# Schatten2021/rust-raytracing

Measured on AMD Instinct MI355X. Metric: Mrays/s (primary rays, whole node), 10k-sphere 1080p 64spp, higher is better.
Workload: dtype f64; 1 GPU; C2: 10k random spheres (scene seed 1), 1920x1080, 64 spp; width=1920, height=1080, rays_per_pixel=64, n_objects=10000, partition=single GPU

## Files before the change

rust-raytracing_amd/csrc/rtx_api.hip:

```cpp
#include "../../include/rtx_hip.h"
#include "rtx_launch.h"

#include <cmath>
#include <cstdio>
#include <cstdlib>
#include <cstring>
#include <string>
#include <thread>
#include <vector>

using namespace rtx;

namespace {

thread_local std::string g_last_error;

int32_t fail(RtxStatus st, const std::string &msg)
{
    g_last_error = msg;
    return (int32_t)st;
}

#define RTX_HIP_CHECK(expr)                                                                              \
    do {                                                                                                 \
// ... 334 lines not shown
        }
        n_in_tree = bvh.tri_order.size();
    } else {
        for (size_t k = 0; k < all_tree.size(); ++k) (all_free[k] == 2 ? demoted : always_recs).push_back(all_tree[k]);
    }
    p.sv.n_tri_tree = (uint32_t)n_in_tree;
    for (const TriRec &r : demoted) { tri32.push_back(r.A); tri32.push_back(r.B); tri_fidx.push_back(r.tri); }
    for (const TriRec &r : always_recs) { tri32.push_back(r.A); tri32.push_back(r.B); tri_fidx.push_back(r.tri); }
    if (!tri32.empty()) {
        tri32.push_back(make_float4(0.f, 0.f, 0.f, 0.f));
        tri32.push_back(make_float4(0.f, 0.f, 0.f, 0.f));
    }
    p.sv.n_tri_filter = (uint32_t)tri_fidx.size();
    p.sv.tri_extent = tri_extent;
    p.sv.n_objects = (uint32_t)n;
    p.sv.n_spheres = (uint32_t)spheres.size();
    p.sv.n_planes = (uint32_t)planes.size();
    p.sv.n_tris = (uint32_t)tris.size();
    for (int c = 0; c < 3; ++c) p.sv.sphere_center[c] = centre[c];
    p.sv.sphere_cmax = cmax;

    p.sv.n_bvh_nodes = (uint32_t)bvh4.nodes.size();
    p.sv.bvh_depth = (uint32_t)bvh4.depth;
    p.sv.bvh_root = bvh4.root;
    p.sv.bvh_origin_limit = (float)bvh.origin_limit;
    p.sv.bvh_inv_max = (float)std::fmin(1.0e30, 1.0e37 / std::fmax(bvh.origin_limit, 1.0));
    p.sv.bvh_flags = (bvh.has_spheres ? 1u : 0u) | (bvh.has_tris ? 2u : 0u) |
                     (bvh.has_tris && !bvh.has_spheres && tree_recs[1].empty() && tree_recs[0].empty() ? 4u : 0u);
    if ((p.sv.bvh_flags & 4u) && build_qnodes(bvh4, p.qnodes)) p.sv.bvh_flags |= 8u;
    else p.qnodes.clear();
#ifndef RTX_LAB
    if ((p.sv.bvh_flags & 12u) == 4u) p.sv.bvh_flags &= ~4u;
#endif
    if ((p.sv.bvh_flags & 3u) == 1u && build_q3nodes(bvh4, bvh.abs_pad, p.q3nodes)) p.sv.bvh_flags |= 16u;
    else p.q3nodes.clear();
    if (debug_prints())
        std::fprintf(stderr, "[rtx_hip] upload: %zu spheres, %zu triangles (%zu in the tree: %zu xy / %zu xz / %zu yz footprints, %zu tested per segment), bvh: %zu binary nodes, %zu wide nodes, depth %d\n",
                     spheres.size(), tris.size(), n_in_tree, tree_recs[2].size(), tree_recs[1].size(), tree_recs[0].size(),
                     demoted.size() + always_recs.size(), bvh.nodes.size(), bvh4.nodes.size(), bvh4.depth);
    std::vector<float4> &leaf32 = p.leaf32;
    leaf32.assign(bvh.prims.size(), make_float4(0.f, 0.f, 0.f, 0.f));
    for (size_t k = 0; k < bvh.prims.size(); ++k) {
        const uint32_t p = bvh.prims[k];
        leaf32[k] = make_float4(fx[p], fy[p], fz[p], fw[p]);
    }
    p.leaf_cr.assign(bvh.prims.size(), make_float4(0.f, 0.f, 0.f, 0.f));
    for (size_t k = 0; k < bvh.prims.size(); ++k) {
        const uint32_t q = bvh.prims[k];
        p.leaf_cr[k] = make_float4(fx[q], fy[q], fz[q], round_up_f32(std::fabs(scene->objects[sphere_id[q]].geom[3])));
    }

    return RTX_OK;
}

int32_t upload_packed(RtxSceneHandle_ *h, const PackedScene &p)
{
    const SceneView sv_before = h->sv;
    std::vector<void *> old_allocs;
    old_allocs.swap(h->scene_allocs);
    {
        SceneView sv = p.sv;
        sv.rays_per_pixel = h->sv.rays_per_pixel; sv.max_bounces = h->sv.max_bounces;
        sv.focal_length = h->sv.focal_length; sv.focal_offset = h->sv.focal_offset; sv.non_focal_offset = h->sv.non_focal_offset;
        sv.seed = h->sv.seed; sv.tuning = h->sv.tuning;
        h->sv = sv;
    }
    h->sv.cam_pos = mk(h->cam.position[0], h->cam.position[1], h->cam.position[2]);
// ... 919 lines not shown
            const Bvh4Node &w = p.bvh4.nodes[k];
            const BvhQNode &q = p.qnodes[k];
            const float lk[4] = { w.b[0].x, w.b[0].y, w.b[0].z, w.b[0].w }, ct[4] = { w.b[1].x, w.b[1].y, w.b[1].z, w.b[1].w };
            for (int c = 0; c < 4; ++c) {
                const uint32_t count = bits(ct[c]), type = q.link[c] >> kQNodeShift;
                if ((count == 0xFFFFFFFFu) != (type == kQNodeEmpty)) return fail(RTX_ERR_INVALID_ARGUMENT, "bvh check: quantised node: empty slot differs");
                if (type == kQNodeEmpty) continue;
                if ((q.link[c] & kQNodeIndexMask) != (bits(lk[c]) & ~kBvhFlatNode) || (type == 0u) != (count == 0u) ||
                    (type != 0u && type != (count & 0xFFFFu)))
                    return fail(RTX_ERR_INVALID_ARGUMENT, "bvh check: quantised node: link / count differs");
                const double lx = (double)q.ox + (double)(q.qx[c] & 0xFFFFu) * q.sx, hx = (double)q.ox + (double)(q.qx[c] >> 16) * q.sx;
                const double ly = (double)q.oy + (double)(q.qy[c] & 0xFFFFu) * q.sy, hy = (double)q.oy + (double)(q.qy[c] >> 16) * q.sy;
                if (!(lx <= (double)w.a[c].x && ly <= (double)w.a[c].y && hx >= (double)w.a[c].z && hy >= (double)w.a[c].w))
                    return fail(RTX_ERR_INVALID_ARGUMENT, "bvh check: quantised rectangle does not contain the child's");
            }
        }
        stats[15] = p.qnodes.size();
    }
    if (p.sv.bvh_flags & 16u) {
        if (p.q3nodes.size() != n_nodes) return fail(RTX_ERR_INVALID_ARGUMENT, "bvh check: 64-byte sphere node count differs");
        for (size_t k = 0; k < n_nodes; ++k) {
            const Bvh4Node &w = p.bvh4.nodes[k];
            const BvhQ3Node &q = p.q3nodes[k];
            const uint32_t *lows[3] = { &q.lox, &q.loy, &q.loz }, *highs[3] = { &q.hix, &q.hiy, &q.hiz };
            const float org[3] = { q.ox, q.oy, q.oz }, stp[3] = { q.sx, q.sy, q.sz };
            for (int c = 0; c < 4; ++c) {
                const uint32_t count = bits(w.b[c].w), type = q.link[c] >> kQNodeShift;
                if ((count == 0xFFFFFFFFu) != (type == kQNodeEmpty)) return fail(RTX_ERR_INVALID_ARGUMENT, "bvh check: 64-byte sphere node: empty slot differs");
                if (type == kQNodeEmpty) continue;
                if ((q.link[c] & kQNodeIndexMask) != bits(w.a[c].w) || (type == 0u) != (count == 0u) || (type != 0u && type != count))
                    return fail(RTX_ERR_INVALID_ARGUMENT, "bvh check: 64-byte sphere node: link / count differs");
                const float l[3] = { w.a[c].x, w.a[c].y, w.a[c].z }, hh[3] = { w.b[c].x, w.b[c].y, w.b[c].z };
                for (int a = 0; a < 3; ++a) {
                    const float dl = std::fmaf((float)((*lows[a] >> (8 * c)) & 255u), stp[a], org[a]);
                    const float dh = std::fmaf((float)((*highs[a] >> (8 * c)) & 255u), stp[a], org[a]);
                    if (!((double)dl <= (double)l[a] - p.bvh.abs_pad * 0.999 && (double)dh >= (double)hh[a] + p.bvh.abs_pad * 0.999))
                        return fail(RTX_ERR_INVALID_ARGUMENT, "bvh check: decoded 64-byte box does not contain the child's (+ pad)");
                }
            }
        }
        stats[15] = p.q3nodes.size();
    }
    if (depth != p.bvh4.depth) return fail(RTX_ERR_INVALID_ARGUMENT, "bvh check: recorded depth differs");
    for (size_t k = 0; k < n_nodes; ++k) if (!node_seen[k]) return fail(RTX_ERR_INVALID_ARGUMENT, "bvh check: unreachable node");
    if ((p.sv.bvh_flags & 1u) && stats[8] != p.spheres.size()) return fail(RTX_ERR_INVALID_ARGUMENT, "bvh check: a sphere is in no leaf");
    if ((p.sv.bvh_flags & 2u) && stats[9] != p.sv.n_tri_tree) return fail(RTX_ERR_INVALID_ARGUMENT, "bvh check: a triangle is in no leaf");
    return RTX_OK;
}

int32_t rtx_debug_paths(RtxSceneHandle h, uint32_t width, uint32_t height, uint32_t row, uint32_t max_steps, RtxPathStep *steps,
                        uint32_t *counts)
{
#ifdef RTX_LAB
    static_assert(sizeof(RtxPathStep) == sizeof(PathStep) && sizeof(PathStep) == 64, "RtxPathStep layout");
    if (!h || !steps || !counts) return fail(RTX_ERR_INVALID_ARGUMENT, "rtx_debug_paths: null argument");
    if (width == 0 || row >= height || max_steps == 0) return fail(RTX_ERR_INVALID_ARGUMENT, "rtx_debug_paths: bad row / size");
    const uint64_t paths = (uint64_t)width * h->cfg.rays_per_pixel;
    if (paths == 0) return RTX_OK;
    if (paths * max_steps > (1ull << 24)) return fail(RTX_ERR_INVALID_ARGUMENT, "rtx_debug_paths: more than 2^24 steps asked for");
    RTX_HIP_CHECK(hipSetDevice(h->device));
    struct Bufs {
        RtxSceneHandle_ *h; double *rgb = nullptr; uint32_t kernel;
        ~Bufs() {
            (void)hipDeviceSynchronize();
            if (h->transcript) (void)hipFree(h->transcript);
            if (h->transcript_counts) (void)hipFree(h->transcript_counts);
            if (rgb) (void)hipFree(rgb);
            h->transcript = nullptr; h->transcript_counts = nullptr; h->transcript_steps = 0; h->cfg.kernel = kernel;
        }
// ... 44 lines not shown
```

rust-raytracing_amd/csrc/rtx_bvh.h:

```cpp
#pragma once

#include <hip/hip_runtime.h>
#include <stdint.h>

#include <algorithm>
#include <cmath>
#include <cstring>
#include <numeric>
#include <vector>

namespace rtx {

struct BvhNode {
    float lo[3];
    uint32_t link;
    float hi[3];
    uint32_t count;
};
static_assert(sizeof(BvhNode) == 32, "BvhNode must be 32 bytes");

constexpr uint32_t kBvhTriLeaf = 0x10000u;
constexpr int kBvhLeafSize = 1;
constexpr int kBvhTriLeafMax = 8;

// ... 376 lines not shown
        }
        BvhQNode q;
        double o[2], sc[2];
        for (int a = 0; a < 2; ++a) {
            o[a] = std::isfinite(lo[a]) ? lo[a] : 0.0;
            const double ext = std::isfinite(lo[a]) ? hi[a] - lo[a] : 0.0;
            sc[a] = ext > 0.0 ? std::exp2(std::ceil(std::log2(ext / 65535.0))) : 1.0;
            while (ext / sc[a] > 65535.0) sc[a] *= 2.0;
            if (!(sc[a] >= 1.1754944e-38 && sc[a] <= 1.0e30)) return false;
        }
        q.ox = (float)o[0]; q.oy = (float)o[1]; q.sx = (float)sc[0]; q.sy = (float)sc[1];
        for (int c = 0; c < 4; ++c) {
            if (ct[c] == 0xFFFFFFFFu) { q.qx[c] = 0x0000FFFFu; q.qy[c] = 0x0000FFFFu; q.link[c] = kQNodeEmpty << kQNodeShift; continue; }
            const double l0 = std::floor(((double)w.a[c].x - o[0]) / sc[0]), h0 = std::ceil(((double)w.a[c].z - o[0]) / sc[0]);
            const double l1 = std::floor(((double)w.a[c].y - o[1]) / sc[1]), h1 = std::ceil(((double)w.a[c].w - o[1]) / sc[1]);
            if (l0 < 0 || l1 < 0 || h0 > 65535 || h1 > 65535) return false;
            q.qx[c] = (uint32_t)l0 | ((uint32_t)h0 << 16);
            q.qy[c] = (uint32_t)l1 | ((uint32_t)h1 << 16);
            uint32_t type;
            if (ct[c] == 0u) type = 0u;
            else if ((ct[c] & kBvhTriLeaf) && (ct[c] & 0xFFFFu) >= 1u && (ct[c] & 0xFFFFu) <= kQNodeLeafMax) type = ct[c] & 0xFFFFu;
            else return false;
            const uint32_t idx = lk[c] & ~kBvhFlatNode;
            if (idx > kQNodeIndexMask) return false;
            if (type == 0u && !(lk[c] & kBvhFlatNode)) return false;
            q.link[c] = (type << kQNodeShift) | idx;
        }
        out.push_back(q);
    }
    return true;
}


struct BvhQ3Node {
    float ox, oy, oz, sx;
    float sy, sz;
    uint32_t lox, loy;
    uint32_t loz, hix, hiy, hiz;
    uint32_t link[4];
};
static_assert(sizeof(BvhQ3Node) == 64, "BvhQ3Node must be 64 bytes");

inline bool build_q3nodes(const Bvh4Build &b4, double abs_pad, std::vector<BvhQ3Node> &out)
{
    out.clear();
    out.reserve(b4.nodes.size());
    auto bits = [](float f) { uint32_t u; std::memcpy(&u, &f, 4); return u; };
    for (const Bvh4Node &w : b4.nodes) {
        double lo[3] = { INFINITY, INFINITY, INFINITY }, hi[3] = { -INFINITY, -INFINITY, -INFINITY };
        uint32_t cnt[4], lnk[4];
        for (int c = 0; c < 4; ++c) {
            cnt[c] = bits(w.b[c].w); lnk[c] = bits(w.a[c].w);
            if (cnt[c] == 0xFFFFFFFFu) continue;
            const float l[3] = { w.a[c].x, w.a[c].y, w.a[c].z }, h[3] = { w.b[c].x, w.b[c].y, w.b[c].z };
            for (int a = 0; a < 3; ++a) {
                if (!std::isfinite(l[a]) || !std::isfinite(h[a])) return false;
                lo[a] = std::min(lo[a], (double)l[a] - abs_pad); hi[a] = std::max(hi[a], (double)h[a] + abs_pad);
            }
        }
        BvhQ3Node q;
        std::memset(&q, 0, sizeof q);
        double o[3], sc[3];
        for (int a = 0; a < 3; ++a) {
            const double ext = std::isfinite(lo[a]) ? hi[a] - lo[a] : 0.0;
            sc[a] = ext > 0.0 ? std::exp2(std::ceil(std::log2(ext / 254.0))) : 1.0;
            if (!(sc[a] >= 1.1754944e-38 && sc[a] <= 1.0e30)) return false;
            o[a] = std::isfinite(lo[a]) ? std::floor(lo[a] / sc[a]) * sc[a] : 0.0;
            while (std::isfinite(lo[a]) && (hi[a] - o[a]) / sc[a] > 255.0) { sc[a] *= 2.0; o[a] = std::floor(lo[a] / sc[a]) * sc[a]; }
            if (!(std::fabs(o[a] / sc[a]) + 256.0 < 16777216.0)) return false;
            if ((double)(float)o[a] != o[a]) return false;
        }
        q.ox = (float)o[0]; q.oy = (float)o[1]; q.oz = (float)o[2]; q.sx = (float)sc[0]; q.sy = (float)sc[1]; q.sz = (float)sc[2];
        uint32_t *lows[3] = { &q.lox, &q.loy, &q.loz }, *highs[3] = { &q.hix, &q.hiy, &q.hiz };
        for (int c = 0; c < 4; ++c) {
            if (cnt[c] == 0xFFFFFFFFu) {
                for (int a = 0; a < 3; ++a) *lows[a] |= 255u << (8 * c);
                q.link[c] = kQNodeEmpty << kQNodeShift;
                continue;
            }
            const float l[3] = { w.a[c].x, w.a[c].y, w.a[c].z }, h[3] = { w.b[c].x, w.b[c].y, w.b[c].z };
            for (int a = 0; a < 3; ++a) {
                const double ql = std::floor(((double)l[a] - abs_pad - o[a]) / sc[a]), qh = std::ceil(((double)h[a] + abs_pad - o[a]) / sc[a]);
                if (ql < 0 || qh > 255 || ql > qh) return false;
                *lows[a] |= (uint32_t)ql << (8 * c);
                *highs[a] |= (uint32_t)qh << (8 * c);
            }
            uint32_t type;
            if (cnt[c] == 0u) type = 0u;
            else if ((cnt[c] & kBvhTriLeaf) == 0u && cnt[c] >= 1u && cnt[c] <= kQNodeLeafMax) type = cnt[c];
            else return false;
            if (lnk[c] > kQNodeIndexMask || (lnk[c] & kBvhFlatNode)) return false;
            q.link[c] = (type << kQNodeShift) | lnk[c];
        }
        out.push_back(q);
    }
    return true;
}

}
```

rust-raytracing_amd/csrc/rtx_bvh_spheres_lab.h:

```cpp
#pragma once

constexpr int kPoolSlots = 128;
constexpr int kPoolStack = kSphStack - 1;
constexpr uint32_t kPoolFresh = 1u << 10, kPoolNoWalk = 1u << 9, kPoolOverflow = 1u << 8;
#ifndef RTX_POOL_SERVE
#define RTX_POOL_SERVE 24
#endif
#ifndef RTX_POOL_WAIT
#define RTX_POOL_WAIT 8
#endif
constexpr uint32_t kPoolWait = RTX_POOL_WAIT;
constexpr uint32_t kPoolServe = RTX_POOL_SERVE;
constexpr int kPoolF64 = 13, kPoolU32 = 28;
struct SphPool {
    double *f;
    uint32_t *u;
    size_t stride;
};

size_t bvh_spheres_pool2_bytes(int n_cus)
{
    const size_t slots = (size_t)n_cus * kSphWavesPerSimd * (kBvhThreads / 64) * kPoolSlots;
    return slots * (kPoolF64 * sizeof(double) + kPoolU32 * sizeof(uint32_t)) + 512;
}
// ... 886 lines not shown
                rec->d = make_double4(__longlong_as_double((long long)r.key),
                                      __longlong_as_double((long long)(((unsigned long long)r.bounce << 32) | (unsigned long long)ridx)), 0.0, 0.0);
                if (nowalk) { sl[9 * kSlotN + my] = kSlotNoWalk; sl[8 * kSlotN + my] = __float_as_uint(__builtin_inff()); }
            } else if (have && !dead) {
                sl[9 * kSlotN + my] = kSlotFresh;
            }
            const bool to_ready = go && !nowalk, to_done = have && !dead && !to_ready;
            const unsigned long long rm = __ballot(to_ready), dm = __ballot(to_done);
            if (to_ready) ready_list[n_ready + bvh_mbcnt(rm)] = (uint8_t)my;
            if (to_done) done_list[n_done + bvh_mbcnt(dm)] = (uint8_t)my;
            n_ready += (uint32_t)__popcll(rm);
            n_done += (uint32_t)__popcll(dm);
#ifndef RTX_SLOT_NOFENCE
            __threadfence_block();
#endif
            { RTX_SLOT_T(t_s2) RTX_SLOT_ACC(2, t_s1, t_s2) }
            continue;
        }
        if (n_idle == 64u) break;
        for (;;) {
            const bool w = walking && node != kNone;
            const bool at_leaf = w && (node >> 29) != 0u;
            const unsigned long long lm = __ballot(at_leaf), am = __ballot(w);
            if (am == 0ull) break;
            if ((uint32_t)__popcll(lm) >= kSphLeafLanes || lm == am) {
                if (at_leaf)
                    sphere_leaf_step_at<STACK, SPILL, kSlotN>(la.sphere_f32, la.sphere_prims, sr, node, sp, &lds_stack[0][0], sl, tid, slot, spill,
                                                              spill_stride, glane, best_up, qcnt, overflow, nleaf);
            } else if (w && !at_leaf) {
#if defined(RTX_LAB) && defined(RTX_SLOT_COUNT_TOP)
                if (node < (uint32_t)(RTX_SLOT_COUNT_TOP)) exact += 1;
#endif
                sphere_node_step_q3<STACK, SPILL>(qnodes, q, node, sp, &lds_stack[0][0], tid, spill, spill_entries, spill_stride, glane, best_up,
                                                  overflow, nbox, kSlotTop > 0 ? (LdsF4Ptr)&lds_top[0] : (LdsF4Ptr) nullptr, top_n);
            }
            const uint32_t n_fin = (uint32_t)__popcll(__ballot(walking && node == kNone));
            if (n_fin >= kSlotWait) break;
        }
        { RTX_SLOT_T(t_s3) RTX_SLOT_ACC(1, t_s1, t_s3) }
    }
#ifdef RTX_SLOT_PROFILE
    exact = sp_prof;
#endif
    unsigned long long box_tests = nbox, filt = (unsigned long long)nbox + nleaf, segs64 = segs;
#pragma unroll
    for (int off = 32; off > 0; off >>= 1) {
        segs64 += __shfl_xor(segs64, off, 64);
        exact += __shfl_xor(exact, off, 64);
        filt += __shfl_xor(filt, off, 64);
        box_tests += __shfl_xor(box_tests, off, 64);
    }
    if (lane == 0) {
        const uint32_t shard = (blockIdx.x * (kBvhThreads >> 6) + (tid >> 6)) & (kCounterShards - 1);
        if (segs64) atomicAdd(&ctr[shard].segments, segs64);
        if (exact) atomicAdd(&ctr[shard].exact_tests, exact);
        if (filt) atomicAdd(&ctr[shard].filter_tests, filt);
        if (box_tests) atomicAdd(&ctr[2 + (shard % (kCounterShards - 2))].pad_, box_tests);
    }
}


static hipError_t launch_sph_lab_stage2(const SceneView *d_sv, const SceneView &sv, const RowsView *d_rv, const RowsView &rv, double *samples,
                                        Counters *counters, uint32_t *spill, uint32_t spill_entries, int n_cus, char *p, uint64_t capacity,
                                        unsigned long long *ctrs, SphQueue &sq, const LeafArrays &la, const float4 *nodes, uint32_t flags,
                                        void *pool_mem, hipStream_t stream)
{
    (void)rv;
// ... 53 lines not shown
```

rust-raytracing_amd/csrc/rtx_kernels.hip:

```cpp
#include "rtx_launch.h"
#include "rtx_traverse.h"

#include <cstdlib>

namespace rtx {

__device__ __forceinline__ uint32_t lane_id() { return __builtin_amdgcn_mbcnt_hi(~0u, __builtin_amdgcn_mbcnt_lo(~0u, 0u)); }

__device__ __forceinline__ uint32_t mbcnt(unsigned long long mask)
{
    return __builtin_amdgcn_mbcnt_hi((uint32_t)(mask >> 32), __builtin_amdgcn_mbcnt_lo((uint32_t)mask, 0u));
}

__device__ __forceinline__ unsigned long long wave_sum_u64(unsigned long long v)
{
#pragma unroll
    for (int off = 32; off > 0; off >>= 1) v += __shfl_xor(v, off, 64);
    return v;
}

__device__ __forceinline__ void flush_counters(Counters *ctr, unsigned long long segs, unsigned long long exact,
                                               unsigned long long filt)
{
    segs = wave_sum_u64(segs);
// ... 487 lines not shown
}

template <class T>
__global__ __launch_bounds__(256) void deinterleave_kernel(const T *__restrict__ parts, T *__restrict__ full,
                                                           uint32_t width, uint32_t height, uint32_t n, uint32_t cap_rows,
                                                           uint32_t block, uint32_t flip)
{
    const uint64_t i = (uint64_t)blockIdx.x * blockDim.x + threadIdx.x;
    const uint64_t row_vals = (uint64_t)width * 3;
    if (i >= row_vals * height) return;
    const uint32_t yo = (uint32_t)(i / row_vals);
    const uint64_t c = i - (uint64_t)yo * row_vals;
    const uint32_t y = flip ? height - 1u - yo : yo;
    const uint32_t b = y / block, p = b % n, k = (b / n) * block + (y - b * block);
    full[i] = parts[((uint64_t)p * cap_rows + k) * row_vals + c];
}

#ifdef RTX_LAB
__global__ void debug_math_kernel(int op, const double *a, const double *b, double *out, uint64_t n)
{
    uint64_t i = (uint64_t)blockIdx.x * blockDim.x + threadIdx.x;
    if (i >= n) return;
    double r;
    switch (op) {
        case 0: r = a[i] / b[i]; break;
        case 1: r = sqrt(a[i]); break;
        case 2: r = sin(a[i]); break;
        case 3: r = cos(a[i]); break;
        case 4: case 5: { double sn, cs; sincos(a[i], &sn, &cs); r = (op == 4) ? sn : cs; } break;
        case 6:
            r = (double)rtx_writelane(__builtin_amdgcn_readfirstlane((int)b[0]), __builtin_amdgcn_readfirstlane((int)b[1]), (int)a[i]);
            break;
        case 9: case 10: { double sn, cs; sincos_2pi(a[i], &sn, &cs); r = (op == 9) ? sn : cs; } break;
        default: {
            double lo, hi;
            rtx_minmax_f64_bits(a[i], b[i], lo, hi);
            r = (op == 7) ? lo : hi;
        } break;
    }
    out[i] = r;
}
#endif

hipError_t launch_trace_exact(const SceneView *d_sv, const RowsView *d_rv, const RowsView &rv, double *samples,
                              Counters *counters, hipStream_t stream)
{
    const uint64_t per_launch = 1ull << 30;
    for (uint64_t off = 0; off < rv.n_rays; off += per_launch) {
        uint64_t n = rv.n_rays - off < per_launch ? rv.n_rays - off : per_launch;
        uint32_t blocks = (uint32_t)((n + 255) / 256);
        hipLaunchKernelGGL(trace_exact_kernel, dim3(blocks), dim3(256), 0, stream, d_sv, d_rv, samples, counters, off);
        hipError_t e = hipGetLastError();
        if (e != hipSuccess) return e;
    }
    return hipSuccess;
}

namespace {

struct MixVariant {
    int s, threads, chunk, q, blocks_per_cu;
    size_t lds;
    const void *fn;
};

template <int S, int T, int CH, int Q, int WPE, int BPC>
// ... 126 lines not shown
```

rust-raytracing_amd/csrc/rtx_traverse.h:

```cpp
#pragma once

#include "rtx_device.h"

namespace rtx {

constexpr int kBvhThreads = 256;
constexpr uint32_t kNone = 0xFFFFFFFFu;
constexpr float kBvhRange64 = 134217728.0f;

struct Ray32 { float ix, iy, iz, nx, ny, nz; };
struct Ray64 { double ix, iy, iz, nx, ny, nz; };
struct Ray32S { float ix, iy, iz, nx, ny, nz, e; };
__device__ __forceinline__ float ray_slack(const Ray32 &) { return 0.0f; }
__device__ __forceinline__ float ray_slack(const Ray32S &r) { return r.e; }

__device__ __forceinline__ void ray32_axis(double o, double dn, double inv_max, float &inv, float &noi)
{
    double i = 1.0 / dn;
    if (!(fabs(i) <= inv_max)) i = copysign(inv_max, dn);
    inv = (float)i;
    noi = (float)(-o * (double)inv);
}

__device__ __forceinline__ void make_ray32(const V3 &pos, const V3 &dirn, double inv_max, Ray32 &r)
// ... 72 lines not shown
}

__device__ __forceinline__ float round_up32(double best)
{
    float b = (float)best;
    if ((double)b < best) b = __uint_as_float(__float_as_uint(b) + (b >= 0.0f ? 1u : 0xFFFFFFFFu));
    return b;
}

typedef float PkF4 __attribute__((ext_vector_type(4)));
typedef const __attribute__((address_space(3))) PkF4 *LdsF4Ptr;
struct PkConst4 {
    const __attribute__((address_space(4))) PkF4 *p;
    __device__ __forceinline__ PkConst4 operator+(size_t i) const { return PkConst4{p + i}; }
    __device__ __forceinline__ float4 operator[](size_t i) const { const PkF4 v = p[i]; return make_float4(v.x, v.y, v.z, v.w); }
};
__device__ __forceinline__ PkConst4 pk_const(const float4 *p) { return PkConst4{(const __attribute__((address_space(4))) PkF4 *)(uintptr_t)p}; }
__device__ __forceinline__ uint32_t pk_bits(float f) { return __builtin_amdgcn_readfirstlane(__float_as_uint(f)); }
struct PkConstU32 {
    const __attribute__((address_space(4))) uint32_t *p;
    __device__ __forceinline__ uint32_t operator[](size_t i) const { return p[i]; }
};
__device__ __forceinline__ PkConstU32 pk_const(const uint32_t *p) { return PkConstU32{(const __attribute__((address_space(4))) uint32_t *)(uintptr_t)p}; }

#if !defined(RTX_WRITELANE_VALIDATED) && defined(__clang_major__)
static_assert(__clang_major__ == 22, "rtx_writelane binds llvm.amdgcn.writelane.i32 by name: validated with AMD clang 22 (ROCm 7.2) only");
#endif
extern "C" __device__ int rtx_writelane(int value, int lane, int old) __asm("llvm.amdgcn.writelane.i32");

__device__ __forceinline__ void rtx_minmax_f64_bits(double a, double b, double &lo, double &hi)
{
    asm("v_min_f64 %0, %1, %2" : "=v"(lo) : "v"(a), "v"(b));
    asm("v_max_f64 %0, %1, %2" : "=v"(hi) : "v"(a), "v"(b));
}

constexpr int kBvhQueue = 8;
constexpr uint32_t kQueueTri = 0x80000000u;

struct LeafArrays {
    const float4 *sphere_f32;
    const uint32_t *sphere_prims;
    const SphereX *spheres;
    const uint32_t *sphere_ids;
    const float4 *tri_f32;
    const uint32_t *tri_fidx;
    const TriX *tris;
};

template <bool TRIS>
__device__ __forceinline__ void flush_candidates(const LeafArrays &la, const RayX &rx, const uint32_t *lds_q, uint32_t tid,
                                                 uint32_t &qcnt, Hit &h, float &best_up, unsigned long long &exact)
{
#pragma unroll 1
    for (uint32_t k = 0; k < qcnt; ++k) {
        const uint32_t idx = lds_q[(size_t)k * kBvhThreads + tid];
        double t;
        if (TRIS && (idx & kQueueTri)) {
            const uint32_t tk = la.tri_fidx[idx & ~kQueueTri];
            if (triangle_distance(la.tris[tk], rx, &t)) hit_consider(h, t, la.tris[tk].id, 2, tk);
        } else {
            if (sphere_distance(la.spheres[idx], rx, &t)) hit_consider(h, t, la.sphere_ids[idx], 0, idx);
        }
    }
    exact += qcnt;
    qcnt = 0;
    if (h.id != kNone) best_up = round_up32(h.t);
// ... 235 lines not shown
    node = key[0] < __builtin_inff() ? lnk[0] : kNone;
    if (node == kNone && sp != 0u) {
        sp -= 1;
        node = (!SPILL || sp < (uint32_t)STACK) ? lds_stack[(size_t)sp * kBvhThreads + tid]
                                                : spill[(size_t)(sp - (uint32_t)STACK) * spill_stride + glane];
    }
}

#ifndef RTX_Q3_SORT64
#define RTX_Q3_SORT64 1
#endif
template <int STACK, bool SPILL, class RAY>
__device__ __forceinline__ void sphere_step_q3(const float4 *__restrict__ qnodes, const float4 *__restrict__ leaf_f32,
                                               const uint32_t *__restrict__ leaf_prims, const RAY &q, const SphereRay &sr,
                                               uint32_t &node, uint32_t &sp, uint32_t *lds_stack, uint32_t *lds_q,
                                               uint32_t tid, uint32_t *__restrict__ spill, uint32_t spill_entries,
                                               size_t spill_stride, size_t glane, float &best_up, uint32_t &qcnt, bool &overflow,
                                               uint32_t &nbox, uint32_t &nleaf)
{
    const float4 *np = qnodes + 4 * (size_t)node;
    const float4 h0 = np[0], h1 = np[1], h2 = np[2], h3 = np[3];
    const float Sx = h0.w * q.ix, Sy = h1.x * q.iy, Sz = h1.y * q.iz;
    const float Ox = __builtin_fmaf(h0.x, q.ix, q.nx), Oy = __builtin_fmaf(h0.y, q.iy, q.ny), Oz = __builtin_fmaf(h0.z, q.iz, q.nz);
    const uint32_t lox = __float_as_uint(h1.z), loy = __float_as_uint(h1.w), loz = __float_as_uint(h2.x);
    const uint32_t hix = __float_as_uint(h2.y), hiy = __float_as_uint(h2.z), hiz = __float_as_uint(h2.w);
    const uint32_t lk[4] = { __float_as_uint(h3.x), __float_as_uint(h3.y), __float_as_uint(h3.z), __float_as_uint(h3.w) };
    const float e = ray_slack(q);
    float tc[4];
    uint32_t lnk[4], typ[4];
    const bool gx = q.ix < 0.0f, gy = q.iy < 0.0f, gz = q.iz < 0.0f;
    const uint32_t nxw = gx ? hix : lox, fxw = gx ? lox : hix;
    const uint32_t nyw = gy ? hiy : loy, fyw = gy ? loy : hiy;
    const uint32_t nzw = gz ? hiz : loz, fzw = gz ? loz : hiz;
#pragma unroll
    for (int c = 0; c < 4; ++c) {
        const float x0 = __builtin_fmaf((float)((nxw >> (8 * c)) & 255u), Sx, Ox), x1 = __builtin_fmaf((float)((fxw >> (8 * c)) & 255u), Sx, Ox);
        const float y0 = __builtin_fmaf((float)((nyw >> (8 * c)) & 255u), Sy, Oy), y1 = __builtin_fmaf((float)((fyw >> (8 * c)) & 255u), Sy, Oy);
        const float z0 = __builtin_fmaf((float)((nzw >> (8 * c)) & 255u), Sz, Oz), z1 = __builtin_fmaf((float)((fzw >> (8 * c)) & 255u), Sz, Oz);
        const float tn = fmaxf(fmaxf(x0, y0), fmaxf(z0, 0.0f));
        const float tf = fminf(fminf(x1, y1), z1);
        const float tn_lo = __builtin_fmaf(tn, 1.0f - 4.76837158e-7f, -e);
        const float tf_hi = __builtin_fmaf(tf, 1.0f + 4.76837158e-7f, e);
        typ[c] = lk[c] >> 29;
        lnk[c] = lk[c] & 0x1FFFFFFFu;
        tc[c] = (tn_lo <= tf_hi && tn_lo <= best_up && typ[c] != 7u) ? tn_lo : __builtin_inff();
    }
    nbox += 4;
    uint32_t leafmask = 0;
#pragma unroll
    for (int c = 0; c < 4; ++c)
        if (tc[c] < __builtin_inff() && typ[c] != 0u) leafmask |= 1u << c;
    while (leafmask != 0u) {
        const uint32_t c = (uint32_t)__builtin_ctz(leafmask);
        leafmask &= leafmask - 1u;
        const uint32_t first = c == 0 ? lnk[0] : (c == 1 ? lnk[1] : (c == 2 ? lnk[2] : lnk[3]));
        const uint32_t n = c == 0 ? typ[0] : (c == 1 ? typ[1] : (c == 2 ? typ[2] : typ[3]));
        for (uint32_t k = 0; k < n; ++k) {
            const float4 rec = leaf_f32[first + k];
            const float ox = rec.x - sr.px, oy = rec.y - sr.py, oz = rec.z - sr.pz;
            const float b = __builtin_fmaf(ox, sr.dx, __builtin_fmaf(oy, sr.dy, oz * sr.dz));
            const float lx = __builtin_fmaf(-b, sr.dx, ox), ly = __builtin_fmaf(-b, sr.dy, oy), lz = __builtin_fmaf(-b, sr.dz, oz);
            const float l2 = __builtin_fmaf(lx, lx, __builtin_fmaf(ly, ly, lz * lz));
            const float Dl = __builtin_fmaf(rec.w, rec.w, -l2);
            const float G = __builtin_fmaf(sr.Kg, rec.w, sr.c0);
            const float Dp = Dl + G;
            if (Dp >= 0.0f) {
                const float tlo = b - __builtin_amdgcn_sqrtf(Dp) * (1.0f + 4.76837158e-7f) - sr.K;
                const float Dm = Dl - G;
                const float thi = Dm > 0.0f ? b - __builtin_amdgcn_sqrtf(Dm) * (1.0f - 4.76837158e-7f) + sr.K : __builtin_inff();
                if (tlo <= best_up && !(thi < 0.0f)) {
                    if (tlo > sr.K) best_up = fminf(best_up, thi);
                    if (qcnt == (uint32_t)kSphQueue) {
                        uint32_t w = 0;
// ... 52 lines not shown
            if (sp < (uint32_t)STACK) { lds_stack[(size_t)sp * kBvhThreads + tid] = (v); sp += 1; } \
            else if (SPILL && sp - (uint32_t)STACK < spill_entries) {                                \
                spill[(size_t)(sp - (uint32_t)STACK) * spill_stride + glane] = (v); sp += 1;         \
            } else overflow = true;                                                                  \
        }
        if (key[3] < __builtin_inff()) RTX_PUSH(lnk[3])
        if (key[2] < __builtin_inff()) RTX_PUSH(lnk[2])
        if (key[1] < __builtin_inff()) RTX_PUSH(lnk[1])
#undef RTX_PUSH
    }
    node = key[0] < __builtin_inff() ? lnk[0] : kNone;
    if (node == kNone && sp != 0u) {
        sp -= 1;
        node = (!SPILL || sp < (uint32_t)STACK) ? lds_stack[(size_t)sp * kBvhThreads + tid]
                                                : spill[(size_t)(sp - (uint32_t)STACK) * spill_stride + glane];
    }
}

template <int STACK, bool SPILL, class RAY>
__device__ __forceinline__ void bvh_traverse_spheres(const float4 *__restrict__ nodes, const float4 *__restrict__ leaf_f32,
                                                     const uint32_t *__restrict__ leaf_prims, const RAY &q, const SphereRay &sr,
                                                     uint32_t root, uint32_t *lds_stack, uint32_t *lds_q,
                                                     uint32_t tid, uint32_t *__restrict__ spill, uint32_t spill_entries,
                                                     size_t spill_stride, size_t glane, float &best_up, uint32_t &qcnt, bool &overflow,
                                                     uint32_t &nbox, uint32_t &nleaf)
{
    uint32_t sp = 0;
    uint32_t node = root;
    while (node != kNone)
        sphere_step<STACK, SPILL>(nodes, leaf_f32, leaf_prims, q, sr, node, sp, lds_stack, lds_q, tid, spill, spill_entries,
                                  spill_stride, glane, best_up, qcnt, overflow, nbox, nleaf);
}

template <int STACK, bool SPILL, class RAY>
__device__ __forceinline__ void sphere_node_step_q3(const float4 *__restrict__ qnodes, const RAY &q, uint32_t &node, uint32_t &sp,
                                                    uint32_t *lds_stack, uint32_t tid, uint32_t *__restrict__ spill,
                                                    uint32_t spill_entries, size_t spill_stride, size_t glane, float best_up,
                                                    bool &overflow, uint32_t &nbox, LdsF4Ptr lds_top = nullptr, uint32_t top_n = 0u)
{
    float4 h0, h1, h2, h3;
    if (lds_top != nullptr && node < top_n) {
        LdsF4Ptr lp = lds_top + 4 * node;
        const PkF4 v0 = lp[0], v1 = lp[1], v2 = lp[2], v3 = lp[3];
        h0 = make_float4(v0.x, v0.y, v0.z, v0.w); h1 = make_float4(v1.x, v1.y, v1.z, v1.w);
        h2 = make_float4(v2.x, v2.y, v2.z, v2.w); h3 = make_float4(v3.x, v3.y, v3.z, v3.w);
    } else {
        const float4 *np = qnodes + 4 * (size_t)node;
        h0 = np[0]; h1 = np[1]; h2 = np[2]; h3 = np[3];
    }
    const float Sx = h0.w * q.ix, Sy = h1.x * q.iy, Sz = h1.y * q.iz;
    const float Ox = __builtin_fmaf(h0.x, q.ix, q.nx), Oy = __builtin_fmaf(h0.y, q.iy, q.ny), Oz = __builtin_fmaf(h0.z, q.iz, q.nz);
    const uint32_t lox = __float_as_uint(h1.z), loy = __float_as_uint(h1.w), loz = __float_as_uint(h2.x);
    const uint32_t hix = __float_as_uint(h2.y), hiy = __float_as_uint(h2.z), hiz = __float_as_uint(h2.w);
    const uint32_t lk[4] = { __float_as_uint(h3.x), __float_as_uint(h3.y), __float_as_uint(h3.z), __float_as_uint(h3.w) };
    const float e = ray_slack(q);
    const bool gx = q.ix < 0.0f, gy = q.iy < 0.0f, gz = q.iz < 0.0f;
    const uint32_t nxw = gx ? hix : lox, fxw = gx ? lox : hix;
    const uint32_t nyw = gy ? hiy : loy, fyw = gy ? loy : hiy;
    const uint32_t nzw = gz ? hiz : loz, fzw = gz ? loz : hiz;
    double kd[4];
#pragma unroll
    for (int c = 0; c < 4; ++c) {
        const float x0 = __builtin_fmaf((float)((nxw >> (8 * c)) & 255u), Sx, Ox), x1 = __builtin_fmaf((float)((fxw >> (8 * c)) & 255u), Sx, Ox);
        const float y0 = __builtin_fmaf((float)((nyw >> (8 * c)) & 255u), Sy, Oy), y1 = __builtin_fmaf((float)((fyw >> (8 * c)) & 255u), Sy, Oy);
        const float z0 = __builtin_fmaf((float)((nzw >> (8 * c)) & 255u), Sz, Oz), z1 = __builtin_fmaf((float)((fzw >> (8 * c)) & 255u), Sz, Oz);
        const float tn = fmaxf(fmaxf(x0, y0), fmaxf(z0, 0.0f));
        const float tf = fminf(fminf(x1, y1), z1);
        const float tn_lo = __builtin_fmaf(tn, 1.0f - 4.76837158e-7f, -e);
        const float tf_hi = __builtin_fmaf(tf, 1.0f + 4.76837158e-7f, e);
        const bool enter = (tn_lo <= fminf(tf_hi, best_up)) & (lk[c] < 0xE0000000u);
        const float key = enter ? tn_lo : __builtin_inff();
        kd[c] = __hiloint2double((int)__float_as_uint(key), (int)lk[c]);
    }
    nbox += 4;
#define RTX_CSWAP(i, j) { double lo_, hi_; rtx_minmax_f64_bits(kd[i], kd[j], lo_, hi_); kd[i] = lo_; kd[j] = hi_; }
    RTX_CSWAP(0, 1) RTX_CSWAP(2, 3) RTX_CSWAP(0, 2) RTX_CSWAP(1, 3) RTX_CSWAP(1, 2)
#undef RTX_CSWAP
    float key[4];
    uint32_t lnk[4];
#pragma unroll
    for (int c = 0; c < 4; ++c) { key[c] = __uint_as_float((uint32_t)__double2hiint(kd[c])); lnk[c] = (uint32_t)__double2loint(kd[c]); }
    const uint32_t npush = (key[1] < __builtin_inff() ? 1u : 0u) + (key[2] < __builtin_inff() ? 1u : 0u) +
                           (key[3] < __builtin_inff() ? 1u : 0u);
    if (sp + 3u <= (uint32_t)STACK) {
#pragma unroll
        for (uint32_t i = 1; i <= 3; ++i) {
            const uint32_t row = i <= npush ? sp + npush - i : (uint32_t)STACK;
            lds_stack[(size_t)row * kBvhThreads + tid] = lnk[i];
        }
        sp += npush;
    } else {
#define RTX_PUSH(v)                                                                                  \
        {                                                                                            \
            if (sp < (uint32_t)STACK) { lds_stack[(size_t)sp * kBvhThreads + tid] = (v); sp += 1; } \
            else if (SPILL && sp - (uint32_t)STACK < spill_entries) {                                \
                spill[(size_t)(sp - (uint32_t)STACK) * spill_stride + glane] = (v); sp += 1;         \
            } else overflow = true;                                                                  \
        }
        if (key[3] < __builtin_inff()) RTX_PUSH(lnk[3])
        if (key[2] < __builtin_inff()) RTX_PUSH(lnk[2])
        if (key[1] < __builtin_inff()) RTX_PUSH(lnk[1])
#undef RTX_PUSH
    }
    node = key[0] < __builtin_inff() ? lnk[0] : kNone;
    if (node == kNone && sp != 0u) {
// ... 51 lines not shown
    nleaf += n;
    node = kNone;
    if (sp != 0u) {
        sp -= 1;
        node = (!SPILL || sp < (uint32_t)STACK) ? lds_stack[(size_t)sp * kBvhThreads + tid]
                                                : spill[(size_t)(sp - (uint32_t)STACK) * spill_stride + glane];
    }
}

template <int STACK, bool SPILL>
__device__ __forceinline__ void sphere_leaf_step(const float4 *__restrict__ leaf_f32, const uint32_t *__restrict__ leaf_prims,
                                                 const SphereRay &sr, uint32_t &node, uint32_t &sp, uint32_t *lds_stack, uint32_t *lds_q,
                                                 uint32_t tid, uint32_t *__restrict__ spill, size_t spill_stride, size_t glane,
                                                 float &best_up, uint32_t &qcnt, bool &overflow, uint32_t &nleaf)
{
    sphere_leaf_step_at<STACK, SPILL, kBvhThreads>(leaf_f32, leaf_prims, sr, node, sp, lds_stack, lds_q, tid, tid, spill, spill_stride, glane,
                                                   best_up, qcnt, overflow, nleaf);
}

#if defined(RTX_LAB) && defined(RTX_SPH_PROFILE)
#define RTX_PROF_ARG , unsigned long long &rtx_prof
#else
#define RTX_PROF_ARG
#endif
template <int STACK, bool SPILL, class RAY>
__device__ __forceinline__ void sphere_walk_phased(const float4 *__restrict__ qnodes, const float4 *__restrict__ leaf_f32,
                                                   const uint32_t *__restrict__ leaf_prims, const RAY &q, const SphereRay &sr,
                                                   uint32_t &node, uint32_t &sp, uint32_t *lds_stack, uint32_t *lds_q,
                                                   uint32_t tid, uint32_t *__restrict__ spill, uint32_t spill_entries,
                                                   size_t spill_stride, size_t glane, float &best_up, uint32_t &qcnt, bool &overflow,
                                                   uint32_t &nbox, uint32_t &nleaf, uint32_t cut_walkers, uint32_t cut_done, uint32_t n_alive,
                                                   uint32_t leaf_lanes RTX_PROF_ARG)
{
    while (node != kNone) {
        const bool at_leaf = (node >> 29) != 0u;
        const unsigned long long lm = __ballot(at_leaf), am = __ballot(true);
#if defined(RTX_LAB) && defined(RTX_SPH_PROFILE)
        {
            const bool leafv = (uint32_t)__popcll(lm) >= leaf_lanes || lm == am;
            const bool leader = (uint32_t)(__ffsll((long long)am) - 1) == (tid & 63u);
            if (RTX_SPH_PROFILE == 3 && !leafv && leader) rtx_prof += 1;
            if (RTX_SPH_PROFILE == 4 && !leafv && !at_leaf) rtx_prof += 1;
            if (RTX_SPH_PROFILE == 5 && leafv && leader) rtx_prof += 1;
            if (RTX_SPH_PROFILE == 6 && leafv && at_leaf) rtx_prof += 1;
            if (RTX_SPH_PROFILE == 7) rtx_prof += 1;
        }
#endif
#if defined(RTX_LAB) && defined(RTX_SPH_PROFILE) && RTX_SPH_PROFILE == 9
        const uint32_t sp_before = sp;
#endif
        if ((uint32_t)__popcll(lm) >= leaf_lanes || lm == am) {
            if (at_leaf)
                sphere_leaf_step<STACK, SPILL>(leaf_f32, leaf_prims, sr, node, sp, lds_stack, lds_q, tid, spill, spill_stride, glane,
                                               best_up, qcnt, overflow, nleaf);
        } else if (!at_leaf) {
            sphere_node_step_q3<STACK, SPILL>(qnodes, q, node, sp, lds_stack, tid, spill, spill_entries, spill_stride, glane, best_up,
                                              overflow, nbox);
        }
#if defined(RTX_LAB) && defined(RTX_SPH_PROFILE) && RTX_SPH_PROFILE == 9
        if (sp_before <= (uint32_t)(RTX_SPH_PROFILE_SP) && sp > (uint32_t)(RTX_SPH_PROFILE_SP)) rtx_prof += 1;
#endif
        const uint32_t still = (uint32_t)__popcll(__ballot(node != kNone));
        if (still < cut_walkers && n_alive - still >= cut_done) break;
    }
}

template <int STACK, bool SPILL, bool Q3, class RAY>
__device__ __forceinline__ void sphere_walk_resumable(const float4 *__restrict__ nodes, const float4 *__restrict__ leaf_f32,
                                                      const uint32_t *__restrict__ leaf_prims, const RAY &q, const SphereRay &sr,
                                                      uint32_t &node, uint32_t &sp, uint32_t *lds_stack, uint32_t *lds_q,
                                                      uint32_t tid, uint32_t *__restrict__ spill, uint32_t spill_entries,
                                                      size_t spill_stride, size_t glane, float &best_up, uint32_t &qcnt, bool &overflow,
                                                      uint32_t &nbox, uint32_t &nleaf, uint32_t cut_walkers, uint32_t cut_done, uint32_t n_alive)
{
    while (node != kNone) {
        if constexpr (Q3)
            sphere_step_q3<STACK, SPILL>(nodes, leaf_f32, leaf_prims, q, sr, node, sp, lds_stack, lds_q, tid, spill, spill_entries,
                                         spill_stride, glane, best_up, qcnt, overflow, nbox, nleaf);
        else
            sphere_step<STACK, SPILL>(nodes, leaf_f32, leaf_prims, q, sr, node, sp, lds_stack, lds_q, tid, spill, spill_entries,
                                      spill_stride, glane, best_up, qcnt, overflow, nbox, nleaf);
        const uint32_t still = (uint32_t)__popcll(__ballot(node != kNone));
        if (still < cut_walkers && n_alive - still >= cut_done) break;
    }
}

template <int STACK, bool SPILL, class RAY>
__device__ __forceinline__ void bvh_traverse_spheres_q3(const float4 *__restrict__ qnodes, const float4 *__restrict__ leaf_f32,
                                                        const uint32_t *__restrict__ leaf_prims, const RAY &q, const SphereRay &sr,
                                                        uint32_t root, uint32_t *lds_stack, uint32_t *lds_q,
// ... 38 lines not shown
```

Baseline: 3609 Mrays/s.

## Decode quantized BVH planes with perm+fma_mix via biased origin, hoist ray slack

Stores the quantized node origin biased by 1024 steps so each 8-bit plane code can be unpacked with v_perm_b32 into an fp16 bit pattern and decoded by v_fma_mix_f32. This replaces a per-plane shift, mask, int-to-float convert and fma. Near and far plane reductions now use max3/min3, and the ray slack widening is hoisted out of the traversal loop into a per-ray constant E. In exchange, the builder enlarges box padding to absorb the larger fp32 rounding error of the biased origin, and rejects nodes whose padding does not converge, so boxes may become slightly looser.

After: 3630 Mrays/s, median of 6. Within noise of the previous version (+0.6%).

```diff
diff --git a/rust-raytracing_amd/csrc/rtx_api.hip b/rust-raytracing_amd/csrc/rtx_api.hip
--- a/rust-raytracing_amd/csrc/rtx_api.hip
+++ b/rust-raytracing_amd/csrc/rtx_api.hip
@@ -390,7 +390,7 @@
 #ifndef RTX_LAB
     if ((p.sv.bvh_flags & 12u) == 4u) p.sv.bvh_flags &= ~4u;
 #endif
-    if ((p.sv.bvh_flags & 3u) == 1u && build_q3nodes(bvh4, bvh.abs_pad, p.q3nodes)) p.sv.bvh_flags |= 16u;
+    if ((p.sv.bvh_flags & 3u) == 1u && build_q3nodes(bvh4, bvh.abs_pad, bvh.origin_limit, p.q3nodes)) p.sv.bvh_flags |= 16u;
     else p.q3nodes.clear();
     if (debug_prints())
         std::fprintf(stderr, "[rtx_hip] upload: %zu spheres, %zu triangles (%zu in the tree: %zu xy / %zu xz / %zu yz footprints, %zu tested per segment), bvh: %zu binary nodes, %zu wide nodes, depth %d\n",
@@ -1376,9 +1376,10 @@
                     return fail(RTX_ERR_INVALID_ARGUMENT, "bvh check: 64-byte sphere node: link / count differs");
                 const float l[3] = { w.a[c].x, w.a[c].y, w.a[c].z }, hh[3] = { w.b[c].x, w.b[c].y, w.b[c].z };
                 for (int a = 0; a < 3; ++a) {
-                    const float dl = std::fmaf((float)((*lows[a] >> (8 * c)) & 255u), stp[a], org[a]);
-                    const float dh = std::fmaf((float)((*highs[a] >> (8 * c)) & 255u), stp[a], org[a]);
-                    if (!((double)dl <= (double)l[a] - p.bvh.abs_pad * 0.999 && (double)dh >= (double)hh[a] + p.bvh.abs_pad * 0.999))
+                    const float dl = std::fmaf((float)(1024u + ((*lows[a] >> (8 * c)) & 255u)), stp[a], org[a]);
+                    const float dh = std::fmaf((float)(1024u + ((*highs[a] >> (8 * c)) & 255u)), stp[a], org[a]);
+                    const double pad = q3_pad(p.bvh.abs_pad, p.bvh.origin_limit, (double)org[a]) * 0.999;
+                    if (!((double)dl <= (double)l[a] - pad && (double)dh >= (double)hh[a] + pad))
                         return fail(RTX_ERR_INVALID_ARGUMENT, "bvh check: decoded 64-byte box does not contain the child's (+ pad)");
                 }
             }
diff --git a/rust-raytracing_amd/csrc/rtx_bvh.h b/rust-raytracing_amd/csrc/rtx_bvh.h
--- a/rust-raytracing_amd/csrc/rtx_bvh.h
+++ b/rust-raytracing_amd/csrc/rtx_bvh.h
@@ -432,6 +432,7 @@
 }
 
 
+constexpr double kQ3Bias = 1024.0;
 struct BvhQ3Node {
     float ox, oy, oz, sx;
     float sy, sz;
@@ -441,13 +442,18 @@
 };
 static_assert(sizeof(BvhQ3Node) == 64, "BvhQ3Node must be 64 bytes");
 
-inline bool build_q3nodes(const Bvh4Build &b4, double abs_pad, std::vector<BvhQ3Node> &out)
+inline double q3_pad(double abs_pad, double origin_limit, double ob)
+{
+    return std::max(abs_pad, (std::fabs(ob) + origin_limit) * (1.0 / 8388608.0));
+}
+
+inline bool build_q3nodes(const Bvh4Build &b4, double abs_pad, double origin_limit, std::vector<BvhQ3Node> &out)
 {
     out.clear();
     out.reserve(b4.nodes.size());
     auto bits = [](float f) { uint32_t u; std::memcpy(&u, &f, 4); return u; };
     for (const Bvh4Node &w : b4.nodes) {
-        double lo[3] = { INFINITY, INFINITY, INFINITY }, hi[3] = { -INFINITY, -INFINITY, -INFINITY };
+        double lo0[3] = { INFINITY, INFINITY, INFINITY }, hi0[3] = { -INFINITY, -INFINITY, -INFINITY };
         uint32_t cnt[4], lnk[4];
         for (int c = 0; c < 4; ++c) {
             cnt[c] = bits(w.b[c].w); lnk[c] = bits(w.a[c].w);
@@ -455,22 +461,34 @@
             const float l[3] = { w.a[c].x, w.a[c].y, w.a[c].z }, h[3] = { w.b[c].x, w.b[c].y, w.b[c].z };
             for (int a = 0; a < 3; ++a) {
                 if (!std::isfinite(l[a]) || !std::isfinite(h[a])) return false;
-                lo[a] = std::min(lo[a], (double)l[a] - abs_pad); hi[a] = std::max(hi[a], (double)h[a] + abs_pad);
+                lo0[a] = std::min(lo0[a], (double)l[a]); hi0[a] = std::max(hi0[a], (double)h[a]);
             }
         }
         BvhQ3Node q;
         std::memset(&q, 0, sizeof q);
-        double o[3], sc[3];
+        double o[3], sc[3], pad[3];
         for (int a = 0; a < 3; ++a) {
-            const double ext = std::isfinite(lo[a]) ? hi[a] - lo[a] : 0.0;
-            sc[a] = ext > 0.0 ? std::exp2(std::ceil(std::log2(ext / 254.0))) : 1.0;
-            if (!(sc[a] >= 1.1754944e-38 && sc[a] <= 1.0e30)) return false;
-            o[a] = std::isfinite(lo[a]) ? std::floor(lo[a] / sc[a]) * sc[a] : 0.0;
-            while (std::isfinite(lo[a]) && (hi[a] - o[a]) / sc[a] > 255.0) { sc[a] *= 2.0; o[a] = std::floor(lo[a] / sc[a]) * sc[a]; }
+            pad[a] = abs_pad;
+            for (int round = 0;; ++round) {
+                const double lo = lo0[a] - pad[a], hi = hi0[a] + pad[a];
+                const double ext = std::isfinite(lo) ? hi - lo : 0.0;
+                sc[a] = ext > 0.0 ? std::exp2(std::ceil(std::log2(ext / 254.0))) : 1.0;
+                if (!(sc[a] >= 1.1754944e-38 && sc[a] <= 1.0e30)) return false;
+                o[a] = std::isfinite(lo) ? std::floor(lo / sc[a]) * sc[a] : 0.0;
+                while (std::isfinite(lo) && (hi - o[a]) / sc[a] > 255.0) { sc[a] *= 2.0; o[a] = std::floor(lo / sc[a]) * sc[a]; }
+                const double need = q3_pad(abs_pad, origin_limit, o[a] - kQ3Bias * sc[a]);
+                if (!std::isfinite(lo) || need <= pad[a]) break;
+                if (round == 4) return false;
+                pad[a] = need * (1.0 + 1.0 / 1024.0);
+            }
+            const double ob = o[a] - kQ3Bias * sc[a];
             if (!(std::fabs(o[a] / sc[a]) + 256.0 < 16777216.0)) return false;
             if ((double)(float)o[a] != o[a]) return false;
-        }
-        q.ox = (float)o[0]; q.oy = (float)o[1]; q.oz = (float)o[2]; q.sx = (float)sc[0]; q.sy = (float)sc[1]; q.sz = (float)sc[2];
+            if (!(std::fabs(ob / sc[a]) + 256.0 < 16777216.0)) return false;
+            if ((double)(float)ob != ob) return false;
+        }
+        q.ox = (float)(o[0] - kQ3Bias * sc[0]); q.oy = (float)(o[1] - kQ3Bias * sc[1]); q.oz = (float)(o[2] - kQ3Bias * sc[2]);
+        q.sx = (float)sc[0]; q.sy = (float)sc[1]; q.sz = (float)sc[2];
         uint32_t *lows[3] = { &q.lox, &q.loy, &q.loz }, *highs[3] = { &q.hix, &q.hiy, &q.hiz };
         for (int c = 0; c < 4; ++c) {
             if (cnt[c] == 0xFFFFFFFFu) {
@@ -480,7 +498,7 @@
             }
             const float l[3] = { w.a[c].x, w.a[c].y, w.a[c].z }, h[3] = { w.b[c].x, w.b[c].y, w.b[c].z };
             for (int a = 0; a < 3; ++a) {
-                const double ql = std::floor(((double)l[a] - abs_pad - o[a]) / sc[a]), qh = std::ceil(((double)h[a] + abs_pad - o[a]) / sc[a]);
+                const double ql = std::floor(((double)l[a] - pad[a] - o[a]) / sc[a]), qh = std::ceil(((double)h[a] + pad[a] - o[a]) / sc[a]);
                 if (ql < 0 || qh > 255 || ql > qh) return false;
                 *lows[a] |= (uint32_t)ql << (8 * c);
                 *highs[a] |= (uint32_t)qh << (8 * c);
diff --git a/rust-raytracing_amd/csrc/rtx_bvh_spheres_lab.h b/rust-raytracing_amd/csrc/rtx_bvh_spheres_lab.h
--- a/rust-raytracing_amd/csrc/rtx_bvh_spheres_lab.h
+++ b/rust-raytracing_amd/csrc/rtx_bvh_spheres_lab.h
@@ -942,7 +942,7 @@
                 if (node < (uint32_t)(RTX_SLOT_COUNT_TOP)) exact += 1;
 #endif
                 sphere_node_step_q3<STACK, SPILL>(qnodes, q, node, sp, &lds_stack[0][0], tid, spill, spill_entries, spill_stride, glane, best_up,
-                                                  overflow, nbox, kSlotTop > 0 ? (LdsF4Ptr)&lds_top[0] : (LdsF4Ptr) nullptr, top_n);
+                                                  q3_widen(ray_slack(q)), overflow, nbox, kSlotTop > 0 ? (LdsF4Ptr)&lds_top[0] : (LdsF4Ptr) nullptr, top_n);
             }
             const uint32_t n_fin = (uint32_t)__popcll(__ballot(walking && node == kNone));
             if (n_fin >= kSlotWait) break;
diff --git a/rust-raytracing_amd/csrc/rtx_kernels.hip b/rust-raytracing_amd/csrc/rtx_kernels.hip
--- a/rust-raytracing_amd/csrc/rtx_kernels.hip
+++ b/rust-raytracing_amd/csrc/rtx_kernels.hip
@@ -543,6 +543,14 @@
             r = (double)rtx_writelane(__builtin_amdgcn_readfirstlane((int)b[0]), __builtin_amdgcn_readfirstlane((int)b[1]), (int)a[i]);
             break;
         case 9: case 10: { double sn, cs; sincos_2pi(a[i], &sn, &cs); r = (op == 9) ? sn : cs; } break;
+        case 11: {
+            const unsigned long long ab = (unsigned long long)__double_as_longlong(a[i]);
+            const float S = __uint_as_float((uint32_t)(ab >> 32)), O = __uint_as_float((uint32_t)__double_as_longlong(b[i]));
+            float t[4];
+            q3_planes((uint32_t)ab, S, O, t);
+            const uint32_t c = (uint32_t)(i & 3u);
+            r = (double)(c == 0 ? t[0] : c == 1 ? t[1] : c == 2 ? t[2] : t[3]);
+        } break;
         default: {
             double lo, hi;
             rtx_minmax_f64_bits(a[i], b[i], lo, hi);
diff --git a/rust-raytracing_amd/csrc/rtx_traverse.h b/rust-raytracing_amd/csrc/rtx_traverse.h
--- a/rust-raytracing_amd/csrc/rtx_traverse.h
+++ b/rust-raytracing_amd/csrc/rtx_traverse.h
@@ -128,6 +128,44 @@
 {
     asm("v_min_f64 %0, %1, %2" : "=v"(lo) : "v"(a), "v"(b));
     asm("v_max_f64 %0, %1, %2" : "=v"(hi) : "v"(a), "v"(b));
+}
+
+__device__ __forceinline__ float rtx_fma_mix_lo(uint32_t h, float s, float o)
+{
+    float r;
+    asm("v_fma_mix_f32 %0, %1, %2, %3 op_sel_hi:[1,0,0]" : "=v"(r) : "v"(h), "v"(s), "v"(o));
+    return r;
+}
+__device__ __forceinline__ float rtx_fma_mix_hi(uint32_t h, float s, float o)
+{
+    float r;
+    asm("v_fma_mix_f32 %0, %1, %2, %3 op_sel:[1,0,0] op_sel_hi:[1,0,0]" : "=v"(r) : "v"(h), "v"(s), "v"(o));
+    return r;
+}
+__device__ __forceinline__ float rtx_near3(float x, float y, float z)
+{
+    float z0, r;
+    asm("v_max_f32 %0, 0, %1" : "=v"(z0) : "v"(z));
+    asm("v_max3_f32 %0, %1, %2, %3" : "=v"(r) : "v"(x), "v"(y), "v"(z0));
+    return r;
+}
+__device__ __forceinline__ float rtx_far3(float x, float y, float z)
+{
+    float r;
+    asm("v_min3_f32 %0, %1, %2, %3" : "=v"(r) : "v"(x), "v"(y), "v"(z));
+    return r;
+}
+template <int PAIR>
+__device__ __forceinline__ void q3_planes2(uint32_t w, float S, float O, float &t0, float &t1)
+{
+    uint32_t h;
+    asm("v_perm_b32 %0, %1, %2, %3" : "=v"(h) : "v"(0x64646464u), "v"(w), "s"(PAIR ? 0x04030402u : 0x04010400u));
+    t0 = rtx_fma_mix_lo(h, S, O); t1 = rtx_fma_mix_hi(h, S, O);
+}
+__device__ __forceinline__ void q3_planes(uint32_t w, float S, float O, float t[4])
+{
+    q3_planes2<0>(w, S, O, t[0], t[1]);
+    q3_planes2<1>(w, S, O, t[2], t[3]);
 }
 
 constexpr int kBvhQueue = 8;
@@ -429,13 +467,13 @@
     const uint32_t nxw = gx ? hix : lox, fxw = gx ? lox : hix;
     const uint32_t nyw = gy ? hiy : loy, fyw = gy ? loy : hiy;
     const uint32_t nzw = gz ? hiz : loz, fzw = gz ? loz : hiz;
+    float xn[4], xf[4], yn[4], yf[4], zn[4], zf[4];
+    q3_planes(nxw, Sx, Ox, xn); q3_planes(fxw, Sx, Ox, xf);
+    q3_planes(nyw, Sy, Oy, yn); q3_planes(fyw, Sy, Oy, yf);
+    q3_planes(nzw, Sz, Oz, zn); q3_planes(fzw, Sz, Oz, zf);
 #pragma unroll
     for (int c = 0; c < 4; ++c) {
-        const float x0 = __builtin_fmaf((float)((nxw >> (8 * c)) & 255u), Sx, Ox), x1 = __builtin_fmaf((float)((fxw >> (8 * c)) & 255u), Sx, Ox);
-        const float y0 = __builtin_fmaf((float)((nyw >> (8 * c)) & 255u), Sy, Oy), y1 = __builtin_fmaf((float)((fyw >> (8 * c)) & 255u), Sy, Oy);
-        const float z0 = __builtin_fmaf((float)((nzw >> (8 * c)) & 255u), Sz, Oz), z1 = __builtin_fmaf((float)((fzw >> (8 * c)) & 255u), Sz, Oz);
-        const float tn = fmaxf(fmaxf(x0, y0), fmaxf(z0, 0.0f));
-        const float tf = fminf(fminf(x1, y1), z1);
+        const float tn = rtx_near3(xn[c], yn[c], zn[c]), tf = rtx_far3(xf[c], yf[c], zf[c]);
         const float tn_lo = __builtin_fmaf(tn, 1.0f - 4.76837158e-7f, -e);
         const float tf_hi = __builtin_fmaf(tf, 1.0f + 4.76837158e-7f, e);
         typ[c] = lk[c] >> 29;
@@ -554,10 +592,11 @@
                                   spill_stride, glane, best_up, qcnt, overflow, nbox, nleaf);
 }
 
+__device__ __forceinline__ float q3_widen(float e) { return e * 0x1.0001p1f + 0x1p-100f; }
 template <int STACK, bool SPILL, class RAY>
 __device__ __forceinline__ void sphere_node_step_q3(const float4 *__restrict__ qnodes, const RAY &q, uint32_t &node, uint32_t &sp,
                                                     uint32_t *lds_stack, uint32_t tid, uint32_t *__restrict__ spill,
-                                                    uint32_t spill_entries, size_t spill_stride, size_t glane, float best_up,
+                                                    uint32_t spill_entries, size_t spill_stride, size_t glane, float best_up, float E,
                                                     bool &overflow, uint32_t &nbox, LdsF4Ptr lds_top = nullptr, uint32_t top_n = 0u)
 {
     float4 h0, h1, h2, h3;
@@ -575,24 +614,29 @@
     const uint32_t lox = __float_as_uint(h1.z), loy = __float_as_uint(h1.w), loz = __float_as_uint(h2.x);
     const uint32_t hix = __float_as_uint(h2.y), hiy = __float_as_uint(h2.z), hiz = __float_as_uint(h2.w);
     const uint32_t lk[4] = { __float_as_uint(h3.x), __float_as_uint(h3.y), __float_as_uint(h3.z), __float_as_uint(h3.w) };
-    const float e = ray_slack(q);
     const bool gx = q.ix < 0.0f, gy = q.iy < 0.0f, gz = q.iz < 0.0f;
     const uint32_t nxw = gx ? hix : lox, fxw = gx ? lox : hix;
     const uint32_t nyw = gy ? hiy : loy, fyw = gy ? loy : hiy;
     const uint32_t nzw = gz ? hiz : loz, fzw = gz ? loz : hiz;
+    const float U = __builtin_fmaf(best_up, 0x1.00002p0f, E);
     double kd[4];
-#pragma unroll
-    for (int c = 0; c < 4; ++c) {
-        const float x0 = __builtin_fmaf((float)((nxw >> (8 * c)) & 255u), Sx, Ox), x1 = __builtin_fmaf((float)((fxw >> (8 * c)) & 255u), Sx, Ox);
-        const float y0 = __builtin_fmaf((float)((nyw >> (8 * c)) & 255u), Sy, Oy), y1 = __builtin_fmaf((float)((fyw >> (8 * c)) & 255u), Sy, Oy);
-        const float z0 = __builtin_fmaf((float)((nzw >> (8 * c)) & 255u), Sz, Oz), z1 = __builtin_fmaf((float)((fzw >> (8 * c)) & 255u), Sz, Oz);
-        const float tn = fmaxf(fmaxf(x0, y0), fmaxf(z0, 0.0f));
-        const float tf = fminf(fminf(x1, y1), z1);
-        const float tn_lo = __builtin_fmaf(tn, 1.0f - 4.76837158e-7f, -e);
-        const float tf_hi = __builtin_fmaf(tf, 1.0f + 4.76837158e-7f, e);
-        const bool enter = (tn_lo <= fminf(tf_hi, best_up)) & (lk[c] < 0xE0000000u);
-        const float key = enter ? tn_lo : __builtin_inff();
+    auto child = [&](int c, float x0, float x1, float y0, float y1, float z0, float z1) {
+        const float tn = rtx_near3(x0, y0, z0), tf = rtx_far3(x1, y1, z1);
+        const float T = __builtin_fmaf(tf, 0x1.00002p0f, E);
+        const bool enter = (tn <= fminf(T, U)) & (lk[c] < 0xE0000000u);
+        const float key = enter ? tn : __builtin_inff();
         kd[c] = __hiloint2double((int)__float_as_uint(key), (int)lk[c]);
+    };
+    {
+        float x0[2], x1[2], y0[2], y1[2], z0[2], z1[2];
+        q3_planes2<0>(nxw, Sx, Ox, x0[0], x0[1]); q3_planes2<0>(fxw, Sx, Ox, x1[0], x1[1]);
+        q3_planes2<0>(nyw, Sy, Oy, y0[0], y0[1]); q3_planes2<0>(fyw, Sy, Oy, y1[0], y1[1]);
+        q3_planes2<0>(nzw, Sz, Oz, z0[0], z0[1]); q3_planes2<0>(fzw, Sz, Oz, z1[0], z1[1]);
+        child(0, x0[0], x1[0], y0[0], y1[0], z0[0], z1[0]); child(1, x0[1], x1[1], y0[1], y1[1], z0[1], z1[1]);
+        q3_planes2<1>(nxw, Sx, Ox, x0[0], x0[1]); q3_planes2<1>(fxw, Sx, Ox, x1[0], x1[1]);
+        q3_planes2<1>(nyw, Sy, Oy, y0[0], y0[1]); q3_planes2<1>(fyw, Sy, Oy, y1[0], y1[1]);
+        q3_planes2<1>(nzw, Sz, Oz, z0[0], z0[1]); q3_planes2<1>(fzw, Sz, Oz, z1[0], z1[1]);
+        child(2, x0[0], x1[0], y0[0], y1[0], z0[0], z1[0]); child(3, x0[1], x1[1], y0[1], y1[1], z0[1], z1[1]);
     }
     nbox += 4;
 #define RTX_CSWAP(i, j) { double lo_, hi_; rtx_minmax_f64_bits(kd[i], kd[j], lo_, hi_); kd[i] = lo_; kd[j] = hi_; }
@@ -710,6 +754,7 @@
                                                    uint32_t &nbox, uint32_t &nleaf, uint32_t cut_walkers, uint32_t cut_done, uint32_t n_alive,
                                                    uint32_t leaf_lanes RTX_PROF_ARG)
 {
+    const float E = q3_widen(ray_slack(q));
     while (node != kNone) {
         const bool at_leaf = (node >> 29) != 0u;
         const unsigned long long lm = __ballot(at_leaf), am = __ballot(true);
@@ -733,7 +778,7 @@
                                                best_up, qcnt, overflow, nleaf);
         } else if (!at_leaf) {
             sphere_node_step_q3<STACK, SPILL>(qnodes, q, node, sp, lds_stack, tid, spill, spill_entries, spill_stride, glane, best_up,
-                                              overflow, nbox);
+                                              E, overflow, nbox);
         }
 #if defined(RTX_LAB) && defined(RTX_SPH_PROFILE) && RTX_SPH_PROFILE == 9
         if (sp_before <= (uint32_t)(RTX_SPH_PROFILE_SP) && sp > (uint32_t)(RTX_SPH_PROFILE_SP)) rtx_prof += 1;
```
